# maciejkula/sbr-rs

Hardware: AMD Instinct MI355X
Metric: train interactions/sec (higher is better)
Workload: dtype f32

## Files before the change

include/sbr_hip.h:

```cpp
#ifndef SBR_HIP_H
#define SBR_HIP_H

#include <stddef.h>
#include <stdint.h>

#ifdef __cplusplus
extern "C" {
#endif

typedef enum sbr_status {
    SBR_OK = 0,
    SBR_ERR_NO_INTERACTIONS = 1,
    SBR_ERR_INVALID_PREDICTION = 2,
    SBR_ERR_INVALID_ARGUMENT = 3,
    SBR_ERR_UNSUPPORTED = 4,
    SBR_ERR_NO_DEVICE = 5,
    SBR_ERR_HIP = 6,
    SBR_ERR_OUT_OF_MEMORY = 7
} sbr_status;

typedef enum sbr_model_kind { SBR_MODEL_LSTM_NORMAL = 0, SBR_MODEL_LSTM_COUPLED = 1, SBR_MODEL_EWMA = 2 } sbr_model_kind;
typedef enum sbr_loss { SBR_LOSS_BPR = 0, SBR_LOSS_HINGE = 1, SBR_LOSS_WARP = 2 } sbr_loss;
typedef enum sbr_optimizer { SBR_OPT_ADAGRAD = 0, SBR_OPT_ADAM = 1 } sbr_optimizer;
typedef enum sbr_parallelism { SBR_PAR_ASYNCHRONOUS = 0, SBR_PAR_SYNCHRONOUS = 1 } sbr_parallelism;
// ... 185 lines not shown
    SBR_K_DENSE_UPDATE = 4,
    SBR_K_SPARSE_UPDATE = 5,
    SBR_K_RANK = 6,
    SBR_K_SPARSE_SORT = 7,
    SBR_K_FAMILIES = 8
} sbr_kernel_family;
sbr_status sbr_model_timing_enable(sbr_model* m, int32_t enable);
sbr_status sbr_model_timing_select(sbr_model* m, uint32_t family_mask);
sbr_status sbr_model_set_overlap(sbr_model* m, int32_t enable);
sbr_status sbr_model_timing_read(sbr_model* m, double* out_ms , uint64_t* out_launches );


sbr_status sbr_set_device(int32_t ordinal);

sbr_status sbr_selftest_math(const float* x, uint64_t n, float* out_cell_h, float* out_sig, float* out_tanh);
sbr_status sbr_selftest_dot_tree(const float* x, const float* y, uint32_t d, uint64_t nrows, float* out);
sbr_status sbr_selftest_mfma(const float* a, const float* b, const float* c0, uint32_t k, float* out,
                             const float* a32, const float* b32, float* out32);
sbr_status sbr_selftest_sort(const uint32_t* rows, uint64_t n, uint32_t row_bits, uint64_t* out_keys, uint32_t* out_head_pos,
                             uint32_t* out_nheads);

#ifdef __cplusplus
}
#endif
#endif
```

sbr_rs_amd/_lib.py:

```python
from __future__ import annotations

import ctypes as C
import os

from ._abi import ABI_VERSION, SbrHparams

_HERE = os.path.dirname(os.path.abspath(__file__))
LIB_PATH = os.environ.get("SBR_HIP_LIB") or os.path.join(_HERE, "libsbr_hip.so")
_lib = None


class EngineUnavailable(RuntimeError):
    """libsbr_hip.so cannot be loaded (not built) — the product path never falls back to CPU."""


def load():
    global _lib
    if _lib is not None:
        return _lib
    if not os.path.exists(LIB_PATH):
        raise EngineUnavailable(
            f"{LIB_PATH} is missing: build it with `python -m sbr_rs_amd.build` (hipcc, gfx950). "
            "There is no CPU fallback.")
    L = C.CDLL(LIB_PATH)
# ... 81 lines not shown
        "sbr_fit_step_owner_reduce_peers": [vp],
        "sbr_fit_step_apply_table_peers": [vp, vp],
        "sbr_model_create_partitioned": [C.POINTER(SbrHparams), C.POINTER(vp)],
        "sbr_partition_num_parts": [vp, u32p],
        "sbr_partition_part_info": [vp, C.c_uint32, u32p, u64p],
        "sbr_partition_export_part": [vp, C.c_uint32, C.POINTER(C.c_int32)],
        "sbr_partition_import_part": [vp, C.c_uint32, C.c_int32],
        "sbr_partition_finalize": [vp],
        "sbr_fit_lists_export": [vp, C.POINTER(C.c_int32), u64p],
        "sbr_fit_lists_import": [vp, C.c_uint32, C.POINTER(C.c_int32), u64p],
        "sbr_fit_step_reduce_own": [vp, C.c_uint64, u32p, vp],
        "sbr_fit_step_owner_apply": [vp, u32p, vp],
        "sbr_fit_step_reduce_own_queued": [vp, C.c_uint64, C.POINTER(vp), vp],
        "sbr_fit_step_owner_apply_queued": [vp, vp, vp],
        "sbr_selftest_math": [vp, C.c_uint64, vp, vp, vp],
        "sbr_selftest_dot_tree": [vp, vp, C.c_uint32, C.c_uint64, vp],
        "sbr_selftest_mfma": [vp, vp, vp, C.c_uint32, vp, vp, vp, vp],
        "sbr_selftest_sort": [vp, C.c_uint64, C.c_uint32, vp, vp, vp],
    }
    for name, args in sig.items():
        fn = getattr(L, name)
        fn.argtypes = args
        fn.restype = C.c_int
    L.sbr_model_destroy.argtypes = [vp]
    L.sbr_model_destroy.restype = None
    L.sbr_fit_plan_destroy.argtypes = [vp]
    L.sbr_fit_plan_destroy.restype = None
    L.sbr_comm_destroy.argtypes = [vp]
    L.sbr_comm_destroy.restype = None
    L.sbr_group_plan_destroy.argtypes = [vp]
# ... 9 lines not shown
    _lib = L
    return L


DECLARED_SYMBOLS = [
    "sbr_model_create", "sbr_model_destroy", "sbr_model_fit", "sbr_fit_begin", "sbr_fit_epoch_prepare",
    "sbr_fit_epoch_prefetch",
    "sbr_fit_step", "sbr_fit_minibatch_rows", "sbr_fit_end", "sbr_fit_end_lagged", "sbr_model_last_fit_lagged_loss", "sbr_fit_counters", "sbr_model_get_rng", "sbr_model_set_rng", "sbr_fit_sparse_stats", "sbr_fit_plan_destroy", "sbr_fit_chunk_bytes", "sbr_fit_dense_bytes",
    "sbr_fit_step_local", "sbr_fit_step_apply", "sbr_fit_step_scatter", "sbr_fit_step_dense", "sbr_fit_step_owner_reduce", "sbr_fit_step_owner_reduce_on", "sbr_fit_step_apply_table", "sbr_fit_step_apply_rows", "sbr_fit_step_apply_dense", "sbr_model_set_stream", "sbr_model_synchronize",
    "sbr_fit_debug_fetch", "sbr_user_representation", "sbr_predict", "sbr_mrr_score", "sbr_model_param_count",
    "sbr_model_get_param", "sbr_model_set_param", "sbr_model_get_param_rows", "sbr_model_get_epoch", "sbr_model_get_counters", "sbr_model_set_counters", "sbr_device_info", "sbr_status_string",
    "sbr_abi_version", "sbr_model_timing_enable", "sbr_model_timing_select", "sbr_model_set_overlap", "sbr_model_timing_read", "sbr_set_device", "sbr_group_fit", "sbr_device_count", "sbr_group_create", "sbr_model_is_partitioned", "sbr_model_create_partitioned", "sbr_partition_num_parts", "sbr_fit_exchange_export", "sbr_fit_exchange_import",
    "sbr_fit_step_scatter_shared", "sbr_fit_step_owner_reduce_peers", "sbr_fit_step_apply_table_peers",
    "sbr_partition_part_info", "sbr_partition_export_part", "sbr_partition_import_part", "sbr_partition_finalize",
    "sbr_fit_lists_export", "sbr_fit_lists_import", "sbr_fit_step_reduce_own", "sbr_fit_step_owner_apply", "sbr_selftest_math",
    "sbr_selftest_dot_tree", "sbr_selftest_mfma", "sbr_selftest_sort", "sbr_release_cached_memory",
    "sbr_group_fit_begin", "sbr_group_epoch_prepare", "sbr_group_step", "sbr_group_step_local", "sbr_group_member_plan",
    "sbr_fit_steps", "sbr_comm_unique_id", "sbr_comm_create", "sbr_comm_destroy", "sbr_fit_step_exchange", "sbr_model_fit_comm", "sbr_model_set_reference_order", "sbr_fit_block_bytes", "sbr_fit_step_apply_blocks_in_order", "sbr_model_set_step_fusion", "sbr_fit_debug_phase_clocks", "sbr_group_synchronize", "sbr_group_plan_set_host_threads", "sbr_group_plan_stats", "sbr_group_fit_end", "sbr_group_plan_destroy",
    "sbr_fit_step_owner_update", "sbr_model_table_slice", "sbr_model_optimizer_state_gathered", "sbr_model_optimizer_state_is_partial",
    "sbr_group_plan_set_exchange", "sbr_group_gather_optimizer_state", "sbr_comm_gather_optimizer_state",
    "sbr_fit_step_reduce_own_queued", "sbr_fit_step_owner_apply_queued",
    "sbr_recommend", "sbr_recommend_reps",
]
```

sbr_rs_amd/csrc/sbr_device.h:

```cpp
#ifndef SBR_DEVICE_H
#define SBR_DEVICE_H

#include <hip/hip_runtime.h>

#include "../../include/sbr_hip.h"
#include "sbr_kernels.h"
#include "sbr_numerics.h"

namespace sbr {

typedef float f32x16 __attribute__((ext_vector_type(16)));

__device__ __forceinline__ float4 ld4(const float* p) { return *reinterpret_cast<const float4*>(p); }
__device__ __forceinline__ void st4(float* p, float4 v) { *reinterpret_cast<float4*>(p) = v; }

typedef unsigned v2u __attribute__((ext_vector_type(2)));
template <int CTRL>
__device__ __forceinline__ float dpp_read(float p) {
    return __uint_as_float(__builtin_amdgcn_update_dpp(0u, __float_as_uint(p), CTRL, 0xF, 0xF, true));
}
template <int L>
__device__ __forceinline__ float group_allreduce(float p) {
    if constexpr (L >= 64) {
        const v2u r = __builtin_amdgcn_permlane32_swap(__float_as_uint(p), __float_as_uint(p), false, false);
// ... 25 lines not shown
    asm volatile("" : "+s"(g));
    return (T*)g;
}

__device__ __forceinline__ float dot4(float4 x, float4 y) {
    float p = x.x * y.x;
    p = sbr_fma(x.y, y.y, p);
    p = sbr_fma(x.z, y.z, p);
    p = sbr_fma(x.w, y.w, p);
    return p;
}

typedef float v2f __attribute__((ext_vector_type(2)));
__device__ __forceinline__ v2f pk_fma(v2f a, v2f b, v2f c) { return __builtin_elementwise_fma(a, b, c); }
__device__ __forceinline__ v2f pk_splat(float x) { return (v2f){x, x}; }
__device__ __forceinline__ void tanh_pq_x2(v2f x, v2f* p, v2f* q) {
    const float cx = __builtin_amdgcn_fmed3f(x.x, -SBR_TANH_CLAMP, SBR_TANH_CLAMP), cy = __builtin_amdgcn_fmed3f(x.y, -SBR_TANH_CLAMP, SBR_TANH_CLAMP);
    x.x = x.x != x.x ? x.x : cx;
    x.y = x.y != x.y ? x.y : cy;
    const v2f x2 = x * x;
    v2f n = pk_splat(-2.76076847742355e-16f);
    n = pk_fma(n, x2, pk_splat(2.00018790482477e-13f));
    n = pk_fma(n, x2, pk_splat(-8.60467152213735e-11f));
    n = pk_fma(n, x2, pk_splat(5.12229709037114e-08f));
    n = pk_fma(n, x2, pk_splat(1.48572235717979e-05f));
    n = pk_fma(n, x2, pk_splat(6.37261928875436e-04f));
    n = pk_fma(n, x2, pk_splat(4.89352455891786e-03f));
    *p = n * x;
    v2f dq = pk_splat(1.19825839466702e-06f);
    dq = pk_fma(dq, x2, pk_splat(1.18534705686654e-04f));
    dq = pk_fma(dq, x2, pk_splat(2.26843463243900e-03f));
    dq = pk_fma(dq, x2, pk_splat(4.89352518554385e-03f));
    *q = dq;
}
// ... 102 lines not shown
```

sbr_rs_amd/csrc/sbr_engine.hip:

```cpp

#include <hip/hip_runtime.h>

#include <algorithm>
#include <array>
#include <atomic>
#include <chrono>
#include <condition_variable>
#include <cmath>
#include <cstdio>
#include <cstdlib>
#include <cstring>
#include <dlfcn.h>
#include <functional>
#include <memory>
#include <mutex>
#include <new>
#include <thread>
#include <unordered_map>
#include <vector>

#include "../../include/sbr_hip.h"
#include "sbr_kernels.h"
#include "sbr_numerics.h"

// ... 470 lines not shown
struct DevicePacked {
    int* off = nullptr;
    int* steps = nullptr;
    int* prev_row = nullptr;
    uint32_t *in_idx = nullptr, *out_idx = nullptr, *ctr = nullptr;
    void release() {
        dfree(off); dfree(steps); dfree(prev_row); dfree(in_idx); dfree(out_idx); dfree(ctr);
        off = steps = prev_row = nullptr;
        in_idx = out_idx = ctr = nullptr;
    }
};

struct WorkBuffers {
    sbr::WorkView v{};
    void release() {
        dfree(v.C); dfree(v.G); dfree(v.dH); dfree(v.dZ); dfree(v.X); dfree(v.zeros); dfree(v.dHrec); dfree(v.dCrec); dfree(v.dab);
        dfree(v.partials); dfree(v.loss); dfree(v.tries); dfree(v.part_loss); dfree(v.part_tries);
        v = sbr::WorkView{};
    }
};

sbr_status alloc_work(const sbr_model* m, uint64_t rmax, uint64_t bmax, bool training, WorkBuffers* wb) {
    const uint64_t d = (uint64_t)m->d;
    sbr::WorkView& v = wb->v;
    v.fold_max_tiles = SBR_FOLD_MAX_TILES_DEFAULT;
    if (m->ng) {
        SBRCHK(dmalloc(&v.C, rmax * d));
        SBRCHK(dmalloc(&v.G, rmax * d * 4));
        SBRCHK(dmalloc(&v.X, rmax * d));
    }
    if (training) {
        SBRCHK(dmalloc(&v.dH, rmax * d));
        SBRCHK(dmalloc(&v.loss, rmax));
        SBRCHK(dmalloc(&v.tries, rmax));
        SBRCHK(dmalloc(&v.part_loss, 2048));
        SBRCHK(dmalloc(&v.part_tries, 2048));
        if (m->ng) {
            const uint64_t rchunk = (rmax + SBR_DW_CHUNK_ROWS - 1) / SBR_DW_CHUNK_ROWS * SBR_DW_CHUNK_ROWS;
            SBRCHK(dmalloc(&v.dZ, rchunk * d * (uint64_t)m->ng));
            v.wide_addresses = std::getenv("SBR_DW_WIDE_ADDRESSES") ? 1 : 0;
            SBRCHK(dmalloc(&v.zeros, 256));
            HIPCHK(hipMemset(v.zeros, 0, 256 * sizeof(float)));
            SBRCHK(dmalloc(&v.dHrec, bmax * d));
            SBRCHK(dmalloc(&v.dCrec, bmax * d));
            const uint64_t nch = (rmax + SBR_DW_CHUNK_ROWS - 1) / SBR_DW_CHUNK_ROWS;
            SBRCHK(dmalloc(&v.partials, nch * dense_count(m)));
        } else {
            SBRCHK(dmalloc(&v.dab, bmax * d));
            SBRCHK(dmalloc(&v.partials, ((bmax + 255) / 256) * d));
        }
    }
    return SBR_OK;
}

// ... 2862 lines not shown
sbr_status sbr_selftest_math(const float* x, uint64_t n, float* out_cell_h, float* out_sig, float* out_tanh) {
    int nd = 0;
    if (hipGetDeviceCount(&nd) != hipSuccess || nd == 0) return SBR_ERR_NO_DEVICE;
    float *dx, *de, *ds, *dt;
    SBRCHK(dmalloc(&dx, n)); SBRCHK(dmalloc(&de, n)); SBRCHK(dmalloc(&ds, n)); SBRCHK(dmalloc(&dt, n));
    HIPCHK(hipMemcpy(dx, x, n * 4, hipMemcpyHostToDevice));
    sbr::launch_selftest_math(dx, de, ds, dt, n, nullptr);
    HIPCHK(hipDeviceSynchronize());
    HIPCHK(hipMemcpy(out_cell_h, de, n * 4, hipMemcpyDeviceToHost));
    HIPCHK(hipMemcpy(out_sig, ds, n * 4, hipMemcpyDeviceToHost));
    HIPCHK(hipMemcpy(out_tanh, dt, n * 4, hipMemcpyDeviceToHost));
    dfree(dx); dfree(de); dfree(ds); dfree(dt);
    return SBR_OK;
}

sbr_status sbr_selftest_dot_tree(const float* x, const float* y, uint32_t d, uint64_t nrows, float* out) {
    int nd = 0;
    if (hipGetDeviceCount(&nd) != hipSuccess || nd == 0) return SBR_ERR_NO_DEVICE;
    if (!dim_ok(d) || nrows == 0) return SBR_ERR_INVALID_ARGUMENT;
    float *dx, *dy, *dout;
    SBRCHK(dmalloc(&dx, nrows * d)); SBRCHK(dmalloc(&dy, nrows * d)); SBRCHK(dmalloc(&dout, nrows));
    HIPCHK(hipMemcpy(dx, x, nrows * d * 4, hipMemcpyHostToDevice));
    HIPCHK(hipMemcpy(dy, y, nrows * d * 4, hipMemcpyHostToDevice));
    sbr::launch_selftest_dot_tree(dx, dy, (int)d, nrows, dout, nullptr);
    HIPCHK(hipDeviceSynchronize());
    HIPCHK(hipMemcpy(out, dout, nrows * 4, hipMemcpyDeviceToHost));
    dfree(dx); dfree(dy); dfree(dout);
    return SBR_OK;
}

// ... 51 lines not shown
```

sbr_rs_amd/csrc/sbr_kernels.h:

```cpp
#ifndef SBR_KERNELS_H
#define SBR_KERNELS_H

#include <hip/hip_runtime.h>
#include <stdint.h>

namespace sbr {

struct MbView {
    int R;
    int B;
    int Tm;
    const int* off;
    const int* steps;
    const int* prev_row;
    const uint32_t* in_idx;
    const uint32_t* out_idx;
    const uint32_t* ctr;
};

struct BlockView {
    uint32_t* header;
    uint32_t* in_idx;
    uint32_t* out_idx;
    uint32_t* neg;
// ... 8 lines not shown
    int coupled;
    uint32_t num_items;
    int loss;
    float lr, l2;
    float *E, *Eacc, *b, *bacc;
    float *W, *Wacc, *bW, *bWacc, *Wp, *WTp;
    float *alpha, *alpha_acc;
    int optimizer;
    float c1, c2;
    float *Em, *bm, *Wm, *bWm, *alpha_m;
};

#define SBR_FOLD_MAX_TILES_DEFAULT 1024
struct WorkView {
    float *C, *G, *dH, *dZ;
    float* X;
    float *dHrec, *dCrec;
    float* dab;
    float* partials;
    float* loss;
    uint32_t* tries;
    double* part_loss;
    unsigned int* part_tries;
    float* zeros;
    int fold_max_tiles;
    int wide_addresses;
    int stream_activations;
};

struct ChunkPtrs {
// ... 116 lines not shown
                             uint32_t capacity, uint64_t* mkeys, uint64_t* mkeys_sorted, void* sort_temp, size_t sort_temp_bytes, hipStream_t s);
void launch_merge_sort(const PeerLists& pl, int ndev, uint32_t total, uint64_t* mkeys, uint64_t* mkeys_sorted, void* sort_temp,
                       size_t sort_temp_bytes, hipStream_t s);
void launch_accumulate_loss(const uint8_t* all_blocks, uint64_t block_bytes, int ndev, double* loss_acc,
                            unsigned long long* ex_acc, hipStream_t s);
void launch_predict(const ModelView& m, const float* user, const uint32_t* items, uint64_t n, float* out, hipStream_t s);
void launch_rank(const ModelView& m, const float* reps, const int* rep_row, uint32_t num_users, const uint32_t* test_item,
                 const uint32_t* test_in_hist, const uint64_t* hist_ptr, const uint32_t* hist_items, float* ts_scratch,
                 uint32_t* ranks, uint32_t* nonfinite_flag, hipStream_t s);
constexpr uint32_t TK_MERGE_MAX = 8192;
uint32_t recommend_groups(uint32_t num_users, uint32_t num_items, uint32_t k, uint32_t* items_per_group);
void launch_recommend(const ModelView& m, const float* reps, const int* rep_row, uint32_t num_users, const uint64_t* excl_ptr,
                      const uint32_t* excl_items, uint32_t k, uint2* lists, uint32_t* lens, uint32_t* out_items, float* out_scores,
                      uint32_t* nonfinite_flag, hipStream_t s);
void launch_selftest_math(const float* x, float* out_cell_h, float* out_sig, float* out_tanh, uint64_t n, hipStream_t s);
void launch_selftest_dot_tree(const float* x, const float* y, int d, uint64_t nrows, float* out, hipStream_t s);
void launch_selftest_mfma_chain(const float* a, const float* b, const float* c0, int k, float* out, hipStream_t s);
void launch_selftest_mfma32_chain(const float* a, const float* b, int k, float* out, hipStream_t s);
void launch_selftest_sort(const uint32_t* rows, uint32_t n, int row_bits, uint64_t* tmp, uint64_t* out, void* temp, uint32_t* head_pos,
                          uint32_t* nheads, hipStream_t s);

}
#endif
```

sbr_rs_amd/csrc/sbr_kernels.hip:

```cpp

#include "sbr_kernels.h"

#include <atomic>
#include <cstdlib>
#include <cstring>

#include "../../include/sbr_hip.h"
#include "sbr_device.h"
#include "sbr_numerics.h"

namespace sbr {

typedef float f32x4 __attribute__((ext_vector_type(4)));
typedef unsigned v4u32 __attribute__((ext_vector_type(4)));

#define EWMA_CHUNK_SEQS 256
#ifndef SBR_FWD_RT
#define SBR_FWD_RT 4
#endif
#ifndef SBR_FWD_WPE
#define SBR_FWD_WPE 3
#endif
#define SBR_MAX_T 1024
#ifndef SBR_FWD_RT4_MIN_TILES
// ... 813 lines not shown
        const int i = e >> 4;
        const int uu = e & 15;
        if (i < nrows) {
            const int u = ut * 16 + uu;
            const size_t r = (size_t)(row_begin + b0 + i);
            const float cprev = t > 0 ? w.C[(size_t)(prev_begin + b0 + i) * D + u] : 0.0f;
            const float* z = &Zs[i * LDZ + uu];
            float zi, zf, zg, zo;
            if (NG == 4) { zi = z[0]; zf = z[16]; zg = z[32]; zo = z[(NG - 1) * 16]; }
            else { zi = 0.0f; zf = z[0]; zg = z[16]; zo = z[32]; }
            float gi, gf, gg, go, cc, hh;
            sbr_lstm_cell_fwd(zi, zf, zg, zo, cprev, NG == 3, &gi, &gf, &gg, &go, &cc, &hh);
            float* G = w.G + r * 4 * D;
            G[u] = gi; G[D + u] = gf; G[2 * D + u] = gg; G[3 * D + u] = go;
            w.C[r * D + u] = cc;
            H[r * D + u] = hh;
        }
    }
}


template <bool COUPLED>
__device__ __forceinline__ void lstm_cell_fwd_x2(v2f zi, v2f zf, v2f zg, v2f zo, v2f c_prev, v2f* gi, v2f* gf, v2f* gg, v2f* go,
                                                  v2f* c, v2f* h) {
    const v2f half = pk_splat(0.5f), one = pk_splat(1.0f);
    v2f pi = pk_splat(0.0f), qi = one, pf, qf, pg, qg, po, qo;
    if (!COUPLED) tanh_pq_x2(half * zi, &pi, &qi);
    tanh_pq_x2(half * zf, &pf, &qf);
    tanh_pq_x2(zg, &pg, &qg);
    tanh_pq_x2(half * zo, &po, &qo);
    const v2f q_if = qi * qf, q_go = qg * qo;
    const v2f den = q_if * q_go;
    const v2f r = (v2f){1.0f / den.x, 1.0f / den.y};
    const v2f r_if = r * q_go, r_go = r * q_if;
    const v2f f = pk_fma(half, pf * (r_if * qi), half);
    const v2f i = COUPLED ? one - f : pk_fma(half, pi * (r_if * qf), half);
    const v2f g = pg * (r_go * qo);
    const v2f o = pk_fma(half, po * (r_go * qg), half);
    const v2f cc = pk_fma(f, c_prev, i * g);
    v2f pc, qc;
    tanh_pq_x2(cc, &pc, &qc);
    const v2f tc = (v2f){pc.x / qc.x, pc.y / qc.y};
    *gi = i; *gf = f; *gg = g; *go = o; *c = cc;
    *h = o * tc;
}

template <int D, int NG, int RT, int UPW>
__global__ __launch_bounds__((D / 16 / UPW) * 64, UPW == 1 ? (RT >= 4 ? 2 : 4) : SBR_FWD_WPE) void lstm_fwd_seq_kernel(ModelView m, MbView mb, float* H, WorkView w, int ntiles) {
    constexpr int K2 = 2 * D;
    constexpr int LDA = K2 + 2;
    constexpr int NS = K2 / 16;
    constexpr int UT = D / 16;
    constexpr int NW = UT / UPW;
    constexpr int NT = NW * 64;
    constexpr int ROWS = 16 * RT;
    constexpr int NV = ROWS * (D / 4);
    constexpr int ITER = (NV + NT - 1) / NT;
    __shared__ float As[ROWS * LDA];
// ... 188 lines not shown
            }
        };
        constexpr bool EARLY_X = RT >= 4 || RT == 1;
        if constexpr (EARLY_X) request_next_x();
        PROF_MARK(3)
        __syncthreads();
        PROF_MARK(4)
        __builtin_amdgcn_s_setprio(3);
        tid = thread_id();
        lane = tid & 63;
        j16 = lane & 15;
        kq = lane >> 4;
        {
            const __amdgpu_buffer_rsrc_t rsG = row_rsrc(w.G, 4 * D, row_begin + b0, nrows);
            const __amdgpu_buffer_rsrc_t rsC = row_rsrc(w.C, D, row_begin + b0, nrows);
            const __amdgpu_buffer_rsrc_t rsH = row_rsrc(H, D, row_begin + b0, nrows);
            const int vG = (kq * 4 * 4 * D + wv * UPW * 16 + j16) * 4;
            const int vC = (kq * 4 * D + wv * UPW * 16 + j16) * 4;
#pragma unroll
            for (int rt = 0; rt < RT; ++rt)
#pragma unroll
                for (int p = 0; p < UPW; ++p) {
                    const int u = (wv * UPW + p) * 16 + j16;
#pragma unroll
                    for (int rp = 0; rp < 4; rp += 2) {
                        v2f zi2, zf2, zg2, zo2;
                        if (NG == 4) {
                            zi2 = (v2f){acc[rt][p][0][rp], acc[rt][p][0][rp + 1]};
                            zf2 = (v2f){acc[rt][p][1][rp], acc[rt][p][1][rp + 1]};
                            zg2 = (v2f){acc[rt][p][2][rp], acc[rt][p][2][rp + 1]};
                            zo2 = (v2f){acc[rt][p][NG - 1][rp], acc[rt][p][NG - 1][rp + 1]};
                        } else {
                            zi2 = pk_splat(0.0f);
                            zf2 = (v2f){acc[rt][p][0][rp], acc[rt][p][0][rp + 1]};
                            zg2 = (v2f){acc[rt][p][1][rp], acc[rt][p][1][rp + 1]};
                            zo2 = (v2f){acc[rt][p][2][rp], acc[rt][p][2][rp + 1]};
                        }
                        v2f gi2, gf2, gg2, go2, cc2, hh2;
                        lstm_cell_fwd_x2<NG == 3>(zi2, zf2, zg2, zo2, (v2f){cst[rt][p][rp], cst[rt][p][rp + 1]}, &gi2, &gf2, &gg2, &go2, &cc2, &hh2);
#pragma unroll
                        for (int e = 0; e < 2; ++e) {
                            const int reg = rp + e;
                            const int i = rt * 16 + kq * 4 + reg;
                            const float gi = gi2[e], gf = gf2[e], gg = gg2[e], go = go2[e], cc = cc2[e], hh = hh2[e];
                            cst[rt][p][reg] = cc;
                            const int sG = ((rt * 16 + reg) * 4 * D + p * 16) * 4, sC = ((rt * 16 + reg) * D + p * 16) * 4;
                            if (stream_act) {
                                __builtin_amdgcn_raw_buffer_store_b32(__builtin_bit_cast(unsigned, gi), rsG, vG, sG, SBR_AUX_FWD_G);
                                __builtin_amdgcn_raw_buffer_store_b32(__builtin_bit_cast(unsigned, gf), rsG, vG + D * 4, sG, SBR_AUX_FWD_G);
                                __builtin_amdgcn_raw_buffer_store_b32(__builtin_bit_cast(unsigned, gg), rsG, vG + 2 * D * 4, sG, SBR_AUX_FWD_G);
                                __builtin_amdgcn_raw_buffer_store_b32(__builtin_bit_cast(unsigned, go), rsG, vG + 3 * D * 4, sG, SBR_AUX_FWD_G);
                                __builtin_amdgcn_raw_buffer_store_b32(__builtin_bit_cast(unsigned, cc), rsC, vC, sC, SBR_AUX_FWD_C);
                            } else {
                                __builtin_amdgcn_raw_buffer_store_b32(__builtin_bit_cast(unsigned, gi), rsG, vG, sG, 0);
                                __builtin_amdgcn_raw_buffer_store_b32(__builtin_bit_cast(unsigned, gf), rsG, vG + D * 4, sG, 0);
                                __builtin_amdgcn_raw_buffer_store_b32(__builtin_bit_cast(unsigned, gg), rsG, vG + 2 * D * 4, sG, 0);
                                __builtin_amdgcn_raw_buffer_store_b32(__builtin_bit_cast(unsigned, go), rsG, vG + 3 * D * 4, sG, 0);
                                __builtin_amdgcn_raw_buffer_store_b32(__builtin_bit_cast(unsigned, cc), rsC, vC, sC, 0);
                            }
                            __builtin_amdgcn_raw_buffer_store_b32(__builtin_bit_cast(unsigned, hh), rsH, vC, sC, 0);
                            As[i * LDA + D + u] = hh;
                        }
                        if constexpr (RT < 4) __builtin_amdgcn_sched_barrier(0);
                    }
                }
        }
        PROF_MARK(5)
        if constexpr (!EARLY_X) request_next_x();
        row_begin = row_begin_next;
        nrows = nrows_next;
        if (more) stage();
        PROF_MARK(0)
    };
// ... 160 lines not shown
        }
    }
    if (!busy) return;
    const int col = ct * 16 + c16;
#pragma unroll
    for (int rt = 0; rt < RT; ++rt)
#pragma unroll
        for (int reg = 0; reg < 4; ++reg) {
            const int i = rt * 16 + kq * 4 + reg;
            if (i < nrows) {
                const int b = b0 + i;
                if (col < D) blk.dX[(size_t)(row_begin + b) * D + col] = acc[rt][reg];
                else w.dHrec[(size_t)b * D + (col - D)] = acc[rt][reg];
            }
        }
}

template <int D, int NG, int RT>
__global__ __launch_bounds__((D / 16) * 64, RT >= 4 ? 2 : 4) void lstm_bwd_seq_kernel(ModelView m, MbView mb, BlockView blk, WorkView w) {
    constexpr int NGD = NG * D;
    constexpr int LDZ = NGD + 2;
    constexpr int NSZ = NGD / 16;
    constexpr int UT = D / 16;
    constexpr int NT = UT * 64;
    constexpr int ROWS = 16 * RT;
    constexpr int Q = D / 4;
    constexpr int CITER = (ROWS * Q) / NT;
#ifndef SBR_BWD_PF_RT1
#define SBR_BWD_PF_RT1 4
#endif
// ... 12 lines not shown
    const int nsteps = mb.steps[b0];
    for (int idx = tid0; idx <= nsteps; idx += NT) s_off[idx] = mb.off[idx];
    for (int idx = tid0; idx < ROWS * D; idx += NT) Zs[(idx / D) * LDZ + (idx % D)] = 0.0f;
    __syncthreads();
    auto step_rows = [&](int t, int* row_begin, int* nrows) {
        const int rb = __builtin_amdgcn_readfirstlane(s_off[t]);
        int nr = __builtin_amdgcn_readfirstlane(s_off[t + 1]) - rb - b0;
        *row_begin = rb;
        *nrows = nr < ROWS ? nr : ROWS;
    };
    float dc[CITER][4];
#pragma unroll
    for (int k = 0; k < CITER; ++k)
#pragma unroll
        for (int j = 0; j < 4; ++j) dc[k][j] = 0.0f;
    float4 pg[CITER][4], pc[CITER], pcp[CITER], pen[CITER], pep[CITER];
    float pcoef[CITER];
    uint32_t nidx[CITER], oidx[CITER];
    auto row_rsrc = [&](const void* base, int row_bytes, int first_row, int live_rows) {
        return __builtin_amdgcn_make_buffer_rsrc((void*)(reinterpret_cast<const char*>(base) + (size_t)first_row * row_bytes), (short)0,
                                                 live_rows * row_bytes, SBR_BUFFER_RSRC_FLAGS);
    };
    static_assert(NT % Q == 0, "item k of a thread is NT / Q rows below item 0, same units");
    auto request_ids = [&](int t) {
        const int tid = thread_id();
        int rb, nr;
        step_rows(t, &rb, &nr);
        const __amdgpu_buffer_rsrc_t rsN = row_rsrc(blk.neg, 4, rb + b0, nr), rsO = row_rsrc(blk.out_idx, 4, rb + b0, nr);
        const int vo = (tid / Q) * 4;
#pragma unroll
        for (int k = 0; k < CITER; ++k) {
// ... 3 lines not shown
    };
    auto request_gathers = [&](int t) {
        const int tid = thread_id();
        int rb, nr;
        step_rows(t, &rb, &nr);
        const float* E = launder(m.E);
        const __amdgpu_buffer_rsrc_t rsK = row_rsrc(blk.coef, 4, rb + b0, nr);
#pragma unroll
        for (int k = 0; k < CITER; ++k) {
            const int u = ((tid + k * NT) % Q) * 4;
            pen[k] = ld4(E + ((size_t)nidx[k] * D + u));
            pep[k] = ld4(E + ((size_t)oidx[k] * D + u));
            pcoef[k] = __builtin_bit_cast(float, __builtin_amdgcn_raw_buffer_load_b32(rsK, (tid / Q) * 4, k * (NT / Q) * 4, 0));
        }
    };
    auto request_cstate = [&](float4* dst, int t) {
        const int tid = thread_id();
        int rb, nr_live;
        step_rows(t, &rb, &nr_live);
        const __amdgpu_buffer_rsrc_t rsC = row_rsrc(w.C, D * 4, rb + b0, nr_live);
#pragma unroll
        for (int k = 0; k < CITER; ++k)
            dst[k] = __builtin_bit_cast(float4, __builtin_amdgcn_raw_buffer_load_b128(rsC, tid * 16, k * NT * 16, SBR_AUX_BWD_LD));
    };
    auto request_gates = [&](int t) {
        const int tid = thread_id();
        int rb, nr;
        step_rows(t, &rb, &nr);
        const __amdgpu_buffer_rsrc_t rsG = row_rsrc(w.G, 4 * D * 4, rb + b0, nr);
        const int vg = (tid / Q) * (4 * D * 4) + (tid % Q) * 16;
#pragma unroll
        for (int k = 0; k < CITER; ++k) {
            const int so = k * (NT / Q) * (4 * D * 4);
#pragma unroll
            for (int g = 0; g < 4; ++g)
                pg[k][g] = __builtin_bit_cast(float4, __builtin_amdgcn_raw_buffer_load_b128(rsG, vg + g * D * 4, so, SBR_AUX_BWD_LD));
        }
    };

    f32x4 ring0[PF], ring1[PF];
    const __amdgpu_buffer_rsrc_t wrs = __builtin_amdgcn_make_buffer_rsrc((void*)m.WTp, (short)0, 2 * D * NGD * 4, SBR_BUFFER_RSRC_FLAGS);
    const uint32_t lane_byte = (uint32_t)(tid0 & 63) * 16u;
    auto load_ring = [&](int slot, int S) {
        ring0[slot] = __builtin_bit_cast(f32x4, __builtin_amdgcn_raw_buffer_load_b128(wrs, lane_byte, (wv * NSZ + S) * 1024, 0));
        ring1[slot] = __builtin_bit_cast(f32x4, __builtin_amdgcn_raw_buffer_load_b128(wrs, lane_byte, ((UT + wv) * NSZ + S) * 1024, 0));
    };
    const int ts = nsteps - 1;
    request_ids(ts);
    request_gates(ts);
    request_cstate(pc, ts);
    request_cstate(pcp, ts > 0 ? ts - 1 : 0);
    request_gathers(ts);
    if (ts > 0) request_ids(ts - 1);
#pragma unroll
    for (int j = 0; j < PF; ++j) load_ring(j, j);

#ifdef SBR_PROF_BWD
    long long bprof[8] = {0, 0, 0, 0, 0, 0, 0, 0};
#define BPROF(k_) { const long long now_ = clock64(); bprof[k_] += now_ - bprof_t; bprof_t = now_; }
    long long bprof_t = clock64();
#else
#define BPROF(k_)
#endif
    auto step = [&](int t) {
        int row_begin, nrows, nrows_above = 0;
        step_rows(t, &row_begin, &nrows);
// ... 9 lines not shown
            for (int k = 0; k < CITER; ++k) {
                const int idx = tid + k * NT;
                const int i = idx / Q;
                const int u = (idx % Q) * 4;
                const bool carried = i < nrows_above;
                const float2 r01 = *reinterpret_cast<const float2*>(&Zs[i * LDZ + u]);
                const float2 r23 = *reinterpret_cast<const float2*>(&Zs[i * LDZ + u + 2]);
                const float recv[4] = {carried ? r01.x : 0.0f, carried ? r01.y : 0.0f, carried ? r23.x : 0.0f, carried ? r23.y : 0.0f};
                const float g_ = pcoef[k];
                const float dhl[4] = {g_ * pen[k].x - g_ * pep[k].x, g_ * pen[k].y - g_ * pep[k].y,
                                      g_ * pen[k].z - g_ * pep[k].z, g_ * pen[k].w - g_ * pep[k].w};
                const float gi[4] = {pg[k][0].x, pg[k][0].y, pg[k][0].z, pg[k][0].w};
                const float gf[4] = {pg[k][1].x, pg[k][1].y, pg[k][1].z, pg[k][1].w};
                const float gg[4] = {pg[k][2].x, pg[k][2].y, pg[k][2].z, pg[k][2].w};
                const float go[4] = {pg[k][3].x, pg[k][3].y, pg[k][3].z, pg[k][3].w};
                const float cc[4] = {pc[k].x, pc[k].y, pc[k].z, pc[k].w};
                const float cp[4] = {pcp[k].x, pcp[k].y, pcp[k].z, pcp[k].w};
                float dz[4][4];
#pragma unroll
                for (int j = 0; j < 4; ++j) {
                    const float dh = dhl[j] + recv[j];
                    float dco;
                    sbr_lstm_cell_bwd(dh, carried ? dc[k][j] : 0.0f, gi[j], gf[j], gg[j], go[j], cc[j], t > 0 ? cp[j] : 0.0f, NG == 3,
                                      &dz[0][j], &dz[1][j], &dz[2][j], &dz[3][j], &dco);
                    dc[k][j] = dco;
                }
#pragma unroll
                for (int g = 0; g < NG; ++g) {
                    const int src = NG == 4 ? g : g + 1;
                    __builtin_amdgcn_raw_buffer_store_b128(__builtin_bit_cast(v4u32, make_float4(dz[src][0], dz[src][1], dz[src][2], dz[src][3])), rsZ,
                                                           vz + g * D * 4, k * (NT / Q) * (NGD * 4), SBR_AUX_BWD_Z);
                    float2* dst = reinterpret_cast<float2*>(&Zs[i * LDZ + g * D + u]);
                    dst[0] = make_float2(dz[src][0], dz[src][1]);
                    dst[1] = make_float2(dz[src][2], dz[src][3]);
                }
            }
        }
        BPROF(2)
        __syncthreads();
// ... 48 lines not shown
#pragma unroll
            for (int j = 0; j < PF; ++j) {
                mma_block(S0 + j, j);
                __builtin_amdgcn_sched_barrier(0);
                load_ring(j, S0 + j + PF);
                __builtin_amdgcn_sched_barrier(0);
            }
        }
#pragma unroll
        for (int j = 0; j < PF; ++j) {
            mma_block(NSZ - PF + j, j);
            __builtin_amdgcn_sched_barrier(0);
        }
        {
            const int tn = t > 0 ? t - 1 : 0;
#pragma unroll
            for (int k = 0; k < CITER; ++k) pc[k] = pcp[k];
            request_gates(tn);
            request_cstate(pcp, tn > 0 ? tn - 1 : 0);
        }
        BPROF(4)
        __syncthreads();
        BPROF(5)
        {
            const __amdgpu_buffer_rsrc_t rsX = row_rsrc(blk.dX, D * 4, row_begin + b0, nrows);
            const int vx = (kq * 4 * D + wv * 16 + c16) * 4;
#pragma unroll
            for (int rt = 0; rt < RT; ++rt)
#pragma unroll
                for (int reg = 0; reg < 4; ++reg) {
                    const int i = rt * 16 + kq * 4 + reg;
                    const float dx = acc[0][rt][reg];
                    __builtin_amdgcn_raw_buffer_store_b32(__builtin_bit_cast(unsigned, dx), rsX, vx, (rt * 16 + reg) * D * 4, SBR_AUX_BWD_ST);
                    Zs[i * LDZ + wv * 16 + c16] = acc[1][rt][reg];
// ... 1063 lines not shown
    for (int q = 0; q < ndev; ++q) {
        const uint32_t* hdr = reinterpret_cast<const uint32_t*>(all_blocks + (size_t)q * block_bytes);
        const double lq = *reinterpret_cast<const double*>(hdr + 4);
        const unsigned long long eq = *reinterpret_cast<const unsigned long long*>(hdr + 6);
        l += lq;
        e += eq;
        tr += hdr[1];
        loss_acc[1 + q] += lq;
        ex_acc[2 + q] += eq;
    }
    loss_acc[0] = l;
    ex_acc[0] = e;
    ex_acc[1] = tr;
}

__global__ void selftest_math_kernel(const float* x, float* e, float* s, float* t, uint64_t n) {
    const uint64_t i = (uint64_t)blockIdx.x * blockDim.x + threadIdx.x;
    if (i >= n) return;
    {
        float gi, gf, gg, go, cc, hh;
        sbr_lstm_cell_fwd(x[i], 0.5f * x[i], -x[i], sbr_fma(0.25f, x[i], 1.0f), 0.5f, 0, &gi, &gf, &gg, &go, &cc, &hh);
        e[i] = hh;
    }
    s[i] = sbr_sigmoidf(x[i]);
    t[i] = sbr_tanhf(x[i]);
}
template <int D>
__global__ void selftest_dot_tree_kernel(const float* x, const float* y, uint64_t nrows, float* out) {
    constexpr int L = D / 4;
    constexpr int GPW = 64 / L;
// ... 463 lines not shown
    if (capacity == 0) return;
    PeerLists pl = pl_in;
    pl.plan = plan;
    hipLaunchKernelGGL(merge_plan_kernel, dim3(1), dim3(64), 0, s, pb, ndev, owner, plan);
    launch_merge_sort(pl, ndev, capacity, mkeys, mkeys_sorted, sort_temp, sort_temp_bytes, s);
    DISPATCH_D(m.d, {
        const int gpb = 4 * (64 / (DD / 4));
        int grid = grid_for_groups((long long)capacity, gpb);
        if (grid > 2048) grid = 2048;
        if (ndev <= 4) hipLaunchKernelGGL((owner_list_apply_kernel<DD, 4>), dim3(grid), dim3(256), 0, s, m, pl, mkeys_sorted);
        else if (ndev <= 8) hipLaunchKernelGGL((owner_list_apply_kernel<DD, 8>), dim3(grid), dim3(256), 0, s, m, pl, mkeys_sorted);
        else hipLaunchKernelGGL((owner_list_apply_kernel<DD, 16>), dim3(grid), dim3(256), 0, s, m, pl, mkeys_sorted);
    });
}

void launch_selftest_math(const float* x, float* out_cell_h, float* out_sig, float* out_tanh, uint64_t n, hipStream_t s) {
    hipLaunchKernelGGL(selftest_math_kernel, dim3((unsigned)((n + 255) / 256)), dim3(256), 0, s, x, out_cell_h, out_sig, out_tanh, n);
}
void launch_selftest_dot_tree(const float* x, const float* y, int d, uint64_t nrows, float* out, hipStream_t s) {
    DISPATCH_D(d, {
        const int gpb = 4 * (64 / (DD / 4));
        hipLaunchKernelGGL((selftest_dot_tree_kernel<DD>), dim3((unsigned)((nrows + gpb - 1) / gpb)), dim3(256), 0, s, x, y, nrows, out);
    });
}
void launch_selftest_mfma_chain(const float* a, const float* b, const float* c0, int k, float* out, hipStream_t s) {
    hipLaunchKernelGGL(selftest_mfma_chain_kernel, dim3(1), dim3(64), 0, s, a, b, c0, k, out);
}
void launch_selftest_mfma32_chain(const float* a, const float* b, int k, float* out, hipStream_t s) {
    hipLaunchKernelGGL(selftest_mfma32_chain_kernel, dim3(1), dim3(64), 0, s, a, b, k, out);
}
// ... 3 lines not shown
```

Measured before the change: 106.4 million.

## Store tanh(c) in forward pass and reuse it in recurrent backward

The LSTM forward kernels now write tanh of the cell state into a new TC buffer, and the recurrent backward kernel loads it instead of recomputing tanh(c). That removes the transcendental from the serial backward step at the cost of one extra store per element in forward and extra memory traffic. The change also swaps the scalar divisions for a packed reciprocal with Newton refinement and a min/max tanh clamp. A selftest kernel sweeps inputs to check these stay bit-exact.

```diff
diff --git a/include/sbr_hip.h b/include/sbr_hip.h
--- a/include/sbr_hip.h
+++ b/include/sbr_hip.h
@@ -223,6 +223,7 @@
 sbr_status sbr_set_device(int32_t ordinal);
 
 sbr_status sbr_selftest_math(const float* x, uint64_t n, float* out_cell_h, float* out_sig, float* out_tanh);
+sbr_status sbr_selftest_cell_sweep(uint64_t* out3);
 sbr_status sbr_selftest_dot_tree(const float* x, const float* y, uint32_t d, uint64_t nrows, float* out);
 sbr_status sbr_selftest_mfma(const float* a, const float* b, const float* c0, uint32_t k, float* out,
                              const float* a32, const float* b32, float* out32);
diff --git a/sbr_rs_amd/_lib.py b/sbr_rs_amd/_lib.py
--- a/sbr_rs_amd/_lib.py
+++ b/sbr_rs_amd/_lib.py
@@ -119,6 +119,7 @@
         "sbr_fit_step_reduce_own_queued": [vp, C.c_uint64, C.POINTER(vp), vp],
         "sbr_fit_step_owner_apply_queued": [vp, vp, vp],
         "sbr_selftest_math": [vp, C.c_uint64, vp, vp, vp],
+        "sbr_selftest_cell_sweep": [vp],
         "sbr_selftest_dot_tree": [vp, vp, C.c_uint32, C.c_uint64, vp],
         "sbr_selftest_mfma": [vp, vp, vp, C.c_uint32, vp, vp, vp, vp],
         "sbr_selftest_sort": [vp, C.c_uint64, C.c_uint32, vp, vp, vp],
@@ -158,7 +159,7 @@
     "sbr_fit_step_scatter_shared", "sbr_fit_step_owner_reduce_peers", "sbr_fit_step_apply_table_peers",
     "sbr_partition_part_info", "sbr_partition_export_part", "sbr_partition_import_part", "sbr_partition_finalize",
     "sbr_fit_lists_export", "sbr_fit_lists_import", "sbr_fit_step_reduce_own", "sbr_fit_step_owner_apply", "sbr_selftest_math",
-    "sbr_selftest_dot_tree", "sbr_selftest_mfma", "sbr_selftest_sort", "sbr_release_cached_memory",
+    "sbr_selftest_cell_sweep", "sbr_selftest_dot_tree", "sbr_selftest_mfma", "sbr_selftest_sort", "sbr_release_cached_memory",
     "sbr_group_fit_begin", "sbr_group_epoch_prepare", "sbr_group_step", "sbr_group_step_local", "sbr_group_member_plan",
     "sbr_fit_steps", "sbr_comm_unique_id", "sbr_comm_create", "sbr_comm_destroy", "sbr_fit_step_exchange", "sbr_model_fit_comm", "sbr_model_set_reference_order", "sbr_fit_block_bytes", "sbr_fit_step_apply_blocks_in_order", "sbr_model_set_step_fusion", "sbr_fit_debug_phase_clocks", "sbr_group_synchronize", "sbr_group_plan_set_host_threads", "sbr_group_plan_stats", "sbr_group_fit_end", "sbr_group_plan_destroy",
     "sbr_fit_step_owner_update", "sbr_model_table_slice", "sbr_model_optimizer_state_gathered", "sbr_model_optimizer_state_is_partial",
diff --git a/sbr_rs_amd/csrc/sbr_device.h b/sbr_rs_amd/csrc/sbr_device.h
--- a/sbr_rs_amd/csrc/sbr_device.h
+++ b/sbr_rs_amd/csrc/sbr_device.h
@@ -63,10 +63,18 @@
 typedef float v2f __attribute__((ext_vector_type(2)));
 __device__ __forceinline__ v2f pk_fma(v2f a, v2f b, v2f c) { return __builtin_elementwise_fma(a, b, c); }
 __device__ __forceinline__ v2f pk_splat(float x) { return (v2f){x, x}; }
+__device__ __forceinline__ float tanh_clamp(float x) {
+    return __builtin_elementwise_minimum(__builtin_elementwise_maximum(x, -SBR_TANH_CLAMP), SBR_TANH_CLAMP);
+}
+__device__ __forceinline__ v2f rcp_den_x2(v2f den) {
+    const v2f one = pk_splat(1.0f), nd = -den;
+    const v2f r0 = (v2f){__builtin_amdgcn_rcpf(den.x), __builtin_amdgcn_rcpf(den.y)};
+    const v2f r = pk_fma(pk_fma(nd, r0, one), r0, r0);
+    const v2f q = pk_fma(pk_fma(nd, r, one), r, r);
+    return pk_fma(pk_fma(nd, q, one), r, q);
+}
 __device__ __forceinline__ void tanh_pq_x2(v2f x, v2f* p, v2f* q) {
-    const float cx = __builtin_amdgcn_fmed3f(x.x, -SBR_TANH_CLAMP, SBR_TANH_CLAMP), cy = __builtin_amdgcn_fmed3f(x.y, -SBR_TANH_CLAMP, SBR_TANH_CLAMP);
-    x.x = x.x != x.x ? x.x : cx;
-    x.y = x.y != x.y ? x.y : cy;
+    x = (v2f){tanh_clamp(x.x), tanh_clamp(x.y)};
     const v2f x2 = x * x;
     v2f n = pk_splat(-2.76076847742355e-16f);
     n = pk_fma(n, x2, pk_splat(2.00018790482477e-13f));
diff --git a/sbr_rs_amd/csrc/sbr_engine.hip b/sbr_rs_amd/csrc/sbr_engine.hip
--- a/sbr_rs_amd/csrc/sbr_engine.hip
+++ b/sbr_rs_amd/csrc/sbr_engine.hip
@@ -508,7 +508,7 @@
 struct WorkBuffers {
     sbr::WorkView v{};
     void release() {
-        dfree(v.C); dfree(v.G); dfree(v.dH); dfree(v.dZ); dfree(v.X); dfree(v.zeros); dfree(v.dHrec); dfree(v.dCrec); dfree(v.dab);
+        dfree(v.C); dfree(v.TC); dfree(v.G); dfree(v.dH); dfree(v.dZ); dfree(v.X); dfree(v.zeros); dfree(v.dHrec); dfree(v.dCrec); dfree(v.dab);
         dfree(v.partials); dfree(v.loss); dfree(v.tries); dfree(v.part_loss); dfree(v.part_tries);
         v = sbr::WorkView{};
     }
@@ -532,6 +532,7 @@
         if (m->ng) {
             const uint64_t rchunk = (rmax + SBR_DW_CHUNK_ROWS - 1) / SBR_DW_CHUNK_ROWS * SBR_DW_CHUNK_ROWS;
             SBRCHK(dmalloc(&v.dZ, rchunk * d * (uint64_t)m->ng));
+            SBRCHK(dmalloc(&v.TC, rmax * d));
             v.wide_addresses = std::getenv("SBR_DW_WIDE_ADDRESSES") ? 1 : 0;
             SBRCHK(dmalloc(&v.zeros, 256));
             HIPCHK(hipMemset(v.zeros, 0, 256 * sizeof(float)));
@@ -3424,6 +3425,17 @@
     return SBR_OK;
 }
 
+sbr_status sbr_selftest_cell_sweep(uint64_t* out3) {
+    int nd = 0;
+    if (hipGetDeviceCount(&nd) != hipSuccess || nd == 0) return SBR_ERR_NO_DEVICE;
+    unsigned long long* dbad;
+    SBRCHK(dmalloc(&dbad, 3));
+    sbr::launch_selftest_cell_sweep(dbad, nullptr);
+    HIPCHK(hipDeviceSynchronize());
+    HIPCHK(hipMemcpy(out3, dbad, 3 * sizeof(unsigned long long), hipMemcpyDeviceToHost));
+    dfree(dbad);
+    return SBR_OK;
+}
 sbr_status sbr_selftest_dot_tree(const float* x, const float* y, uint32_t d, uint64_t nrows, float* out) {
     int nd = 0;
     if (hipGetDeviceCount(&nd) != hipSuccess || nd == 0) return SBR_ERR_NO_DEVICE;
diff --git a/sbr_rs_amd/csrc/sbr_kernels.h b/sbr_rs_amd/csrc/sbr_kernels.h
--- a/sbr_rs_amd/csrc/sbr_kernels.h
+++ b/sbr_rs_amd/csrc/sbr_kernels.h
@@ -46,6 +46,7 @@
 #define SBR_FOLD_MAX_TILES_DEFAULT 1024
 struct WorkView {
     float *C, *G, *dH, *dZ;
+    float* TC;
     float* X;
     float *dHrec, *dCrec;
     float* dab;
@@ -192,6 +193,7 @@
                       const uint32_t* excl_items, uint32_t k, uint2* lists, uint32_t* lens, uint32_t* out_items, float* out_scores,
                       uint32_t* nonfinite_flag, hipStream_t s);
 void launch_selftest_math(const float* x, float* out_cell_h, float* out_sig, float* out_tanh, uint64_t n, hipStream_t s);
+void launch_selftest_cell_sweep(unsigned long long* bad, hipStream_t s);
 void launch_selftest_dot_tree(const float* x, const float* y, int d, uint64_t nrows, float* out, hipStream_t s);
 void launch_selftest_mfma_chain(const float* a, const float* b, const float* c0, int k, float* out, hipStream_t s);
 void launch_selftest_mfma32_chain(const float* a, const float* b, int k, float* out, hipStream_t s);
diff --git a/sbr_rs_amd/csrc/sbr_kernels.hip b/sbr_rs_amd/csrc/sbr_kernels.hip
--- a/sbr_rs_amd/csrc/sbr_kernels.hip
+++ b/sbr_rs_amd/csrc/sbr_kernels.hip
@@ -851,6 +851,7 @@
             float* G = w.G + r * 4 * D;
             G[u] = gi; G[D + u] = gf; G[2 * D + u] = gg; G[3 * D + u] = go;
             w.C[r * D + u] = cc;
+            if (w.TC) w.TC[r * D + u] = sbr_tanhf(cc);
             H[r * D + u] = hh;
         }
     }
@@ -859,7 +860,7 @@
 
 template <bool COUPLED>
 __device__ __forceinline__ void lstm_cell_fwd_x2(v2f zi, v2f zf, v2f zg, v2f zo, v2f c_prev, v2f* gi, v2f* gf, v2f* gg, v2f* go,
-                                                  v2f* c, v2f* h) {
+                                                  v2f* c, v2f* tch, v2f* h) {
     const v2f half = pk_splat(0.5f), one = pk_splat(1.0f);
     v2f pi = pk_splat(0.0f), qi = one, pf, qf, pg, qg, po, qo;
     if (!COUPLED) tanh_pq_x2(half * zi, &pi, &qi);
@@ -868,7 +869,7 @@
     tanh_pq_x2(half * zo, &po, &qo);
     const v2f q_if = qi * qf, q_go = qg * qo;
     const v2f den = q_if * q_go;
-    const v2f r = (v2f){1.0f / den.x, 1.0f / den.y};
+    const v2f r = rcp_den_x2(den);
     const v2f r_if = r * q_go, r_go = r * q_if;
     const v2f f = pk_fma(half, pf * (r_if * qi), half);
     const v2f i = COUPLED ? one - f : pk_fma(half, pi * (r_if * qf), half);
@@ -878,7 +879,7 @@
     v2f pc, qc;
     tanh_pq_x2(cc, &pc, &qc);
     const v2f tc = (v2f){pc.x / qc.x, pc.y / qc.y};
-    *gi = i; *gf = f; *gg = g; *go = o; *c = cc;
+    *gi = i; *gf = f; *gg = g; *go = o; *c = cc; *tch = tc;
     *h = o * tc;
 }
 
@@ -1097,6 +1098,7 @@
         {
             const __amdgpu_buffer_rsrc_t rsG = row_rsrc(w.G, 4 * D, row_begin + b0, nrows);
             const __amdgpu_buffer_rsrc_t rsC = row_rsrc(w.C, D, row_begin + b0, nrows);
+            const __amdgpu_buffer_rsrc_t rsTC = row_rsrc(w.TC, D, row_begin + b0, w.TC ? nrows : 0);
             const __amdgpu_buffer_rsrc_t rsH = row_rsrc(H, D, row_begin + b0, nrows);
             const int vG = (kq * 4 * 4 * D + wv * UPW * 16 + j16) * 4;
             const int vC = (kq * 4 * D + wv * UPW * 16 + j16) * 4;
@@ -1119,13 +1121,14 @@
                             zg2 = (v2f){acc[rt][p][1][rp], acc[rt][p][1][rp + 1]};
                             zo2 = (v2f){acc[rt][p][2][rp], acc[rt][p][2][rp + 1]};
                         }
-                        v2f gi2, gf2, gg2, go2, cc2, hh2;
-                        lstm_cell_fwd_x2<NG == 3>(zi2, zf2, zg2, zo2, (v2f){cst[rt][p][rp], cst[rt][p][rp + 1]}, &gi2, &gf2, &gg2, &go2, &cc2, &hh2);
+                        v2f gi2, gf2, gg2, go2, cc2, tc2, hh2;
+                        lstm_cell_fwd_x2<NG == 3>(zi2, zf2, zg2, zo2, (v2f){cst[rt][p][rp], cst[rt][p][rp + 1]}, &gi2, &gf2, &gg2, &go2, &cc2, &tc2,
+                                                  &hh2);
 #pragma unroll
                         for (int e = 0; e < 2; ++e) {
                             const int reg = rp + e;
                             const int i = rt * 16 + kq * 4 + reg;
-                            const float gi = gi2[e], gf = gf2[e], gg = gg2[e], go = go2[e], cc = cc2[e], hh = hh2[e];
+                            const float gi = gi2[e], gf = gf2[e], gg = gg2[e], go = go2[e], cc = cc2[e], tc = tc2[e], hh = hh2[e];
                             cst[rt][p][reg] = cc;
                             const int sG = ((rt * 16 + reg) * 4 * D + p * 16) * 4, sC = ((rt * 16 + reg) * D + p * 16) * 4;
                             if (stream_act) {
@@ -1134,12 +1137,14 @@
                                 __builtin_amdgcn_raw_buffer_store_b32(__builtin_bit_cast(unsigned, gg), rsG, vG + 2 * D * 4, sG, SBR_AUX_FWD_G);
                                 __builtin_amdgcn_raw_buffer_store_b32(__builtin_bit_cast(unsigned, go), rsG, vG + 3 * D * 4, sG, SBR_AUX_FWD_G);
                                 __builtin_amdgcn_raw_buffer_store_b32(__builtin_bit_cast(unsigned, cc), rsC, vC, sC, SBR_AUX_FWD_C);
+                                __builtin_amdgcn_raw_buffer_store_b32(__builtin_bit_cast(unsigned, tc), rsTC, vC, sC, SBR_AUX_FWD_C);
                             } else {
                                 __builtin_amdgcn_raw_buffer_store_b32(__builtin_bit_cast(unsigned, gi), rsG, vG, sG, 0);
                                 __builtin_amdgcn_raw_buffer_store_b32(__builtin_bit_cast(unsigned, gf), rsG, vG + D * 4, sG, 0);
                                 __builtin_amdgcn_raw_buffer_store_b32(__builtin_bit_cast(unsigned, gg), rsG, vG + 2 * D * 4, sG, 0);
                                 __builtin_amdgcn_raw_buffer_store_b32(__builtin_bit_cast(unsigned, go), rsG, vG + 3 * D * 4, sG, 0);
                                 __builtin_amdgcn_raw_buffer_store_b32(__builtin_bit_cast(unsigned, cc), rsC, vC, sC, 0);
+                                __builtin_amdgcn_raw_buffer_store_b32(__builtin_bit_cast(unsigned, tc), rsTC, vC, sC, 0);
                             }
                             __builtin_amdgcn_raw_buffer_store_b32(__builtin_bit_cast(unsigned, hh), rsH, vC, sC, 0);
                             As[i * LDA + D + u] = hh;
@@ -1330,6 +1335,26 @@
                 else w.dHrec[(size_t)b * D + (col - D)] = acc[rt][reg];
             }
         }
+}
+
+
+__device__ __forceinline__ void lstm_cell_bwd_tc(float dh, float dc_in, float i, float f, float g, float o, float tc, float c_prev, int coupled,
+                                                 float* dzi, float* dzf, float* dzg, float* dzo, float* dc_out) {
+    const float d_o = dh * tc;
+    const float dc = sbr_fma(dh * o, 1.0f - tc * tc, dc_in);
+    const float di = dc * g;
+    const float dg = dc * i;
+    float df = dc * c_prev;
+    *dc_out = dc * f;
+    if (coupled) {
+        df = df - di;
+        *dzi = 0.0f;
+    } else {
+        *dzi = di * (i * (1.0f - i));
+    }
+    *dzf = df * (f * (1.0f - f));
+    *dzg = dg * (1.0f - g * g);
+    *dzo = d_o * (o * (1.0f - o));
 }
 
 template <int D, int NG, int RT>
@@ -1372,7 +1397,7 @@
     for (int k = 0; k < CITER; ++k)
 #pragma unroll
         for (int j = 0; j < 4; ++j) dc[k][j] = 0.0f;
-    float4 pg[CITER][4], pc[CITER], pcp[CITER], pen[CITER], pep[CITER];
+    float4 pg[CITER][4], ptc[CITER], pcp[CITER], pen[CITER], pep[CITER];
     float pcoef[CITER];
     uint32_t nidx[CITER], oidx[CITER];
     auto row_rsrc = [&](const void* base, int row_bytes, int first_row, int live_rows) {
@@ -1406,11 +1431,11 @@
             pcoef[k] = __builtin_bit_cast(float, __builtin_amdgcn_raw_buffer_load_b32(rsK, (tid / Q) * 4, k * (NT / Q) * 4, 0));
         }
     };
-    auto request_cstate = [&](float4* dst, int t) {
+    auto request_cstate = [&](const float* rows, float4* dst, int t) {
         const int tid = thread_id();
         int rb, nr_live;
         step_rows(t, &rb, &nr_live);
-        const __amdgpu_buffer_rsrc_t rsC = row_rsrc(w.C, D * 4, rb + b0, nr_live);
+        const __amdgpu_buffer_rsrc_t rsC = row_rsrc(rows, D * 4, rb + b0, nr_live);
 #pragma unroll
         for (int k = 0; k < CITER; ++k)
             dst[k] = __builtin_bit_cast(float4, __builtin_amdgcn_raw_buffer_load_b128(rsC, tid * 16, k * NT * 16, SBR_AUX_BWD_LD));
@@ -1440,8 +1465,8 @@
     const int ts = nsteps - 1;
     request_ids(ts);
     request_gates(ts);
-    request_cstate(pc, ts);
-    request_cstate(pcp, ts > 0 ? ts - 1 : 0);
+    request_cstate(w.TC, ptc, ts);
+    request_cstate(w.C, pcp, ts > 0 ? ts - 1 : 0);
     request_gathers(ts);
     if (ts > 0) request_ids(ts - 1);
 #pragma unroll
@@ -1481,15 +1506,15 @@
                 const float gf[4] = {pg[k][1].x, pg[k][1].y, pg[k][1].z, pg[k][1].w};
                 const float gg[4] = {pg[k][2].x, pg[k][2].y, pg[k][2].z, pg[k][2].w};
                 const float go[4] = {pg[k][3].x, pg[k][3].y, pg[k][3].z, pg[k][3].w};
-                const float cc[4] = {pc[k].x, pc[k].y, pc[k].z, pc[k].w};
+                const float tc[4] = {ptc[k].x, ptc[k].y, ptc[k].z, ptc[k].w};
                 const float cp[4] = {pcp[k].x, pcp[k].y, pcp[k].z, pcp[k].w};
                 float dz[4][4];
 #pragma unroll
                 for (int j = 0; j < 4; ++j) {
                     const float dh = dhl[j] + recv[j];
                     float dco;
-                    sbr_lstm_cell_bwd(dh, carried ? dc[k][j] : 0.0f, gi[j], gf[j], gg[j], go[j], cc[j], t > 0 ? cp[j] : 0.0f, NG == 3,
-                                      &dz[0][j], &dz[1][j], &dz[2][j], &dz[3][j], &dco);
+                    lstm_cell_bwd_tc(dh, carried ? dc[k][j] : 0.0f, gi[j], gf[j], gg[j], go[j], tc[j], t > 0 ? cp[j] : 0.0f, NG == 3,
+                                     &dz[0][j], &dz[1][j], &dz[2][j], &dz[3][j], &dco);
                     dc[k][j] = dco;
                 }
 #pragma unroll
@@ -1568,10 +1593,9 @@
         }
         {
             const int tn = t > 0 ? t - 1 : 0;
-#pragma unroll
-            for (int k = 0; k < CITER; ++k) pc[k] = pcp[k];
             request_gates(tn);
-            request_cstate(pcp, tn > 0 ? tn - 1 : 0);
+            request_cstate(w.TC, ptc, tn);
+            request_cstate(w.C, pcp, tn > 0 ? tn - 1 : 0);
         }
         BPROF(4)
         __syncthreads();
@@ -2665,6 +2689,45 @@
     ex_acc[1] = tr;
 }
 
+__global__ void selftest_cell_sweep_kernel(unsigned long long* bad) {
+    const uint64_t stride = (uint64_t)gridDim.x * blockDim.x, i0 = (uint64_t)blockIdx.x * blockDim.x + threadIdx.x;
+    auto same = [](float a, float b) { return (a != a && b != b) || __float_as_uint(a) == __float_as_uint(b); };
+    unsigned long long nb_tanh = 0, nb_rcp = 0, n_rcp = 0;
+    for (uint64_t b = 2 * i0; b < (1ull << 32); b += 2 * stride) {
+        const v2f x = (v2f){__uint_as_float((uint32_t)b), __uint_as_float((uint32_t)b + 1u)};
+        v2f p, q;
+        tanh_pq_x2(x, &p, &q);
+#pragma unroll
+        for (int e = 0; e < 2; ++e) {
+            float pr, qr;
+            sbr_tanh_pq(x[e], &pr, &qr);
+            nb_tanh += !(same(p[e], pr) && same(q[e], qr));
+        }
+    }
+    const uint32_t lo = 0x2f800000u , hi = 0x3f800000u ;
+    for (uint64_t b = lo + 2 * i0; b <= hi; b += 2 * stride) {
+        const uint32_t b1 = (uint32_t)b + 1u <= hi ? (uint32_t)b + 1u : (uint32_t)b;
+        const v2f x = (v2f){__uint_as_float((uint32_t)b), __uint_as_float(b1)};
+        const v2f r = rcp_den_x2(x);
+        nb_rcp += !same(r.x, 1.0f / x.x);
+        nb_rcp += !same(r.y, 1.0f / x.y);
+        n_rcp += 2;
+    }
+    if (i0 == 0) {
+        const uint32_t nans[4] = {0x7fc00000u, 0x7f800001u, 0xffc00000u, 0x7fffffffu};
+#pragma unroll
+        for (int k = 0; k < 4; k += 2) {
+            const v2f x = (v2f){__uint_as_float(nans[k]), __uint_as_float(nans[k + 1])};
+            const v2f r = rcp_den_x2(x);
+            nb_rcp += !same(r.x, 1.0f / x.x);
+            nb_rcp += !same(r.y, 1.0f / x.y);
+            n_rcp += 2;
+        }
+    }
+    atomicAdd(&bad[0], nb_tanh);
+    atomicAdd(&bad[1], nb_rcp);
+    atomicAdd(&bad[2], n_rcp);
+}
 __global__ void selftest_math_kernel(const float* x, float* e, float* s, float* t, uint64_t n) {
     const uint64_t i = (uint64_t)blockIdx.x * blockDim.x + threadIdx.x;
     if (i >= n) return;
@@ -3158,6 +3221,10 @@
     });
 }
 
+void launch_selftest_cell_sweep(unsigned long long* bad, hipStream_t s) {
+    (void)hipMemsetAsync(bad, 0, 3 * sizeof(unsigned long long), s);
+    hipLaunchKernelGGL(selftest_cell_sweep_kernel, dim3(4096), dim3(256), 0, s, bad);
+}
 void launch_selftest_math(const float* x, float* out_cell_h, float* out_sig, float* out_tanh, uint64_t n, hipStream_t s) {
     hipLaunchKernelGGL(selftest_math_kernel, dim3((unsigned)((n + 255) / 256)), dim3(256), 0, s, x, out_cell_h, out_sig, out_tanh, n);
 }
```

Result: no change. 106.2 million, median of 3 (-0.2%).
